# google-research/sparf

Measured on AMD Instinct MI355X. Metric: training rays/sec (64c+128f samples, 8x256 MLP), higher is better.
Workload: dtype bf16x3; 1 GPU; BASELINE configs[1]: DTU-shaped scene, fixed GT poses, photometric loss; 4 views 300x400, 4096 rays x (64 coarse + 128 fine) per GPU and step, fwd+bwd+clip+Adam, both 8x256 MLPs; samples=64+128, precision_mode=bf16x3, launch=eager, optimizer=clip_grad_norm(0.1) + Adam, sparf_amd.optim.FusedAdam

## Files before the change

sparf_amd/csrc/mlp_dev.h:

```cpp
#pragma once
#include <hip/hip_runtime.h>

#include <utility>

#include "streams.h"

namespace sparf {

typedef __bf16 bf16x8 __attribute__((ext_vector_type(8)));
typedef float f32x16 __attribute__((ext_vector_type(16)));
typedef float f32x4 __attribute__((ext_vector_type(4)));
typedef unsigned int u32x4 __attribute__((ext_vector_type(4)));

#define SP_DEV __device__ __forceinline__

template <int N, class F, int... I>
SP_DEV void static_for_impl(F&& f, std::integer_sequence<int, I...>) {
    (f(std::integral_constant<int, I>{}), ...);
}
template <int N, class F> SP_DEV void static_for(F&& f) {
    static_for_impl<N>(static_cast<F&&>(f), std::make_integer_sequence<int, N>{});
}

template <int PREC> struct Policy;

template <> struct Policy<PREC_BF16> {
    enum { PREC = PREC_BF16, KJ = 8, CH = 8, FRAG_BYTES = 1024, LANE_BYTES = 16, G = group_g(PREC_BF16), NWAVES = nwaves_of(PREC_BF16), PREFETCH = 4 };
    typedef bf16x8 B;
    typedef bf16x8 A;
    typedef __bf16 act_t;
    typedef __bf16 stage_t;
    static SP_DEV B zero() { B z; for (int i = 0; i < 8; ++i) z[i] = (__bf16)0.0f; return z; }
    static SP_DEV A lds_frag(const char* p) { return *(const bf16x8*)p; }
    enum { NPART = 1 };
    template <int PART> static SP_DEV f32x16 mfma_part(const A& a, const B& b, f32x16 c) { return __builtin_amdgcn_mfma_f32_32x32x16_bf16(a, b, c, 0, 0, 0); }
    static SP_DEV void set(B* v, int q, float x) { v[q >> 3][q & 7] = (__bf16)x; }
    static SP_DEV float get(const B* v, int q) { return (float)v[q >> 3][q & 7]; }
};

template <> struct Policy<PREC_FP32> {
    enum { PREC = PREC_FP32, KJ = 1, CH = 4, FRAG_BYTES = 256, LANE_BYTES = 4, G = group_g(PREC_FP32), NWAVES = nwaves_of(PREC_FP32), PREFETCH = 4 };
    typedef float B;
    typedef float A;
    typedef float act_t;
    typedef float stage_t;
    static SP_DEV B zero() { return 0.0f; }
    static SP_DEV A lds_frag(const char* p) { return *(const float*)p; }
    enum { NPART = 1 };
    template <int PART> static SP_DEV f32x16 mfma_part(const A& a, const B& b, f32x16 c) { return __builtin_amdgcn_mfma_f32_32x32x2f32(a, b, c, 0, 0, 0); }
    static SP_DEV void set(B* v, int q, float x) { v[q] = x; }
    static SP_DEV float get(const B* v, int q) { return v[q]; }
};

struct bfpair { bf16x8 hi, lo; };
#ifndef SP_X3_PREFETCH
#define SP_X3_PREFETCH 4
#endif
template <> struct Policy<PREC_X3> {
    enum { PREC = PREC_X3, KJ = 8, CH = 8, FRAG_BYTES = 2048, LANE_BYTES = 16, G = group_g(PREC_X3), NWAVES = nwaves_of(PREC_X3), PREFETCH = SP_X3_PREFETCH };
    typedef bfpair B;
    typedef bfpair A;
    typedef __bf16 act_t;
    typedef float stage_t;
    static SP_DEV B zero() { B z; for (int i = 0; i < 8; ++i) { z.hi[i] = (__bf16)0.0f; z.lo[i] = (__bf16)0.0f; } return z; }
    static SP_DEV A lds_frag(const char* p) { A a; a.hi = *(const bf16x8*)p; a.lo = *(const bf16x8*)(p + 1024); return a; }
    enum { NPART = 3 };
    template <int PART> static SP_DEV f32x16 mfma_part(const A& a, const B& b, f32x16 c) {
        if constexpr (PART == 0) return __builtin_amdgcn_mfma_f32_32x32x16_bf16(a.lo, b.hi, c, 0, 0, 0);
        else if constexpr (PART == 1) return __builtin_amdgcn_mfma_f32_32x32x16_bf16(a.hi, b.lo, c, 0, 0, 0);
        else return __builtin_amdgcn_mfma_f32_32x32x16_bf16(a.hi, b.hi, c, 0, 0, 0);
    }
    static SP_DEV void set(B* v, int q, float x) {
        const __bf16 h = (__bf16)x;
        v[q >> 3].hi[q & 7] = h;
        v[q >> 3].lo[q & 7] = (__bf16)(x - (float)h);
    }
    static SP_DEV float get(const B* v, int q) { return (float)v[q >> 3].hi[q & 7] + (float)v[q >> 3].lo[q & 7]; }
};

#ifndef SP_X3_DGRAD_PARTS
#define SP_X3_DGRAD_PARTS 2
#endif
#ifndef SP_X3_DGRAD_WAVES
#define SP_X3_DGRAD_WAVES 0
#endif
template <int W> struct PolicyX3DgradT {
    enum { PREC = PREC_X3, KJ = 8, CH = 8, FRAG_BYTES = 2048, LANE_BYTES = 16, G = group_g(PREC_X3), NWAVES = W,
#ifdef SP_X3_DGRAD_PREFETCH
           PREFETCH = SP_X3_DGRAD_PREFETCH,
#else
           PREFETCH = (W == 8 ? 3 : 4),
#endif
           NPART = SP_X3_DGRAD_PARTS };
    typedef bf16x8 B;
    typedef bfpair A;
    typedef __bf16 act_t;
    typedef float stage_t;
    static SP_DEV B zero() { B z; for (int i = 0; i < 8; ++i) z[i] = (__bf16)0.0f; return z; }
    static SP_DEV A lds_frag(const char* p) { A a; a.hi = *(const bf16x8*)p; a.lo = *(const bf16x8*)(p + 1024); return a; }
    template <int PART> static SP_DEV f32x16 mfma_part(const A& a, const B& b, f32x16 c) {
        if constexpr (PART == 0 && NPART == 2) return __builtin_amdgcn_mfma_f32_32x32x16_bf16(a.lo, b, c, 0, 0, 0);
        else return __builtin_amdgcn_mfma_f32_32x32x16_bf16(a.hi, b, c, 0, 0, 0);
    }
    static SP_DEV void set(B* v, int q, float x) { v[q >> 3][q & 7] = (__bf16)x; }
    static SP_DEV float get(const B* v, int q) { return (float)v[q >> 3][q & 7]; }
};
typedef PolicyX3DgradT<8> PolicyX3Dgrad;
typedef PolicyX3DgradT<4> PolicyX3DgradW4;

#ifdef SP_PROF
struct Prof {
    unsigned long long last, acc[10];
    SP_DEV void start() { for (int i = 0; i < 10; ++i) acc[i] = 0; last = __builtin_amdgcn_s_memtime(); }
    SP_DEV void lap(int k) { const unsigned long long now = __builtin_amdgcn_s_memtime(); acc[k] += now - last; last = now; }
};
#define SP_LAP(prof, k) (prof).lap(k)
#else
struct Prof { SP_DEV void start() {} };
#define SP_LAP(prof, k) ((void)0)
#endif

enum { PIPE_LDS_BYTES = 2 * CHUNK_MAX_BYTES };
#ifdef SP_PROBE_NO_DMA
#define SP_PROBE_NBYTES(x) 0
#else
#define SP_PROBE_NBYTES(x) (x)
#endif

template <int NWAVES, bool SPREAD = false> struct WeightPipe {
    __amdgpu_buffer_rsrc_t rsrc;
    char* lds;
    int wave, lane16;
    unsigned parity;
    Prof prof;

    SP_DEV void init(const char* g, unsigned stream_bytes, char* l) {
        prof.start();
        rsrc = __builtin_amdgcn_make_buffer_rsrc((void*)g, 0, stream_bytes, 0x00020000);
        lane16 = (threadIdx.x & 63) * 16;
        lds = l;
        wave = __builtin_amdgcn_readfirstlane(threadIdx.x >> 6);
        parity = 0;
    }
    SP_DEV void fetch(int off, int bytes, unsigned buf) {
        char* dst = lds + buf * CHUNK_MAX_BYTES;
#pragma unroll
        for (int i = 0; i < CHUNK_MAX_BYTES / (NWAVES * 1024); ++i) {
            int o = (i * NWAVES + wave) * 1024;
            if (o < bytes)
                __builtin_amdgcn_raw_ptr_buffer_load_lds(rsrc, (__attribute__((address_space(3))) void*)(dst + o), 16,
                                                         lane16, off + o, 0, 0);
        }
    }
    template <int OFF, int BYTES, int I> SP_DEV void fetch_piece(unsigned buf) {
        if constexpr (I * NWAVES * 1024 < BYTES) {
            const int o = (I * NWAVES + wave) * 1024;
            if ((I + 1) * NWAVES * 1024 <= BYTES || o < BYTES) {
                __builtin_amdgcn_raw_ptr_buffer_load_lds(rsrc, (__attribute__((address_space(3))) void*)(lds + buf * CHUNK_MAX_BYTES + o), 16,
                                                         lane16, OFF + o, 0, 0);
            }
        }
    }
    enum { PIECES = CHUNK_MAX_BYTES / (NWAVES * 1024), IS_SPREAD = SPREAD };
    SP_DEV void prime(int off, int bytes) { fetch(off, bytes, parity); }
    SP_DEV void drain() { __syncthreads(); }
    template <int NOFF, int NBYTES> SP_DEV const char* acquire() {
#ifndef SP_PROBE_NO_BARRIER
        __syncthreads();
#endif
        SP_LAP(prof, 0);
        if constexpr (!SPREAD)
            static_for<PIECES>([&](auto ic) { this->template fetch_piece<NOFF, NBYTES, decltype(ic)::value>(parity ^ 1u); });
        SP_LAP(prof, 1);
        const char* cur = lds + parity * CHUNK_MAX_BYTES;
        parity ^= 1u;
        return cur;
    }
};

struct NoMid { template <class I, class N> SP_DEV void operator()(I, N) const {} };
#ifndef SP_SPREAD_NUM
#define SP_SPREAD_NUM 3
#define SP_SPREAD_DEN 4
#endif
#ifndef SP_SLOT_BALANCE
#define SP_SLOT_BALANCE 1
#endif
SP_DEV constexpr int last_part_slot(int t, int nmb, int npart) { return (t / nmb) * (npart * nmb) + (npart - 1) * nmb + t % nmb; }
template <class Pipe, int NOFF, int NBYTES, int NMB = 1, int NPART = 1> struct SpreadFetch {
    Pipe& pipe;
    template <class I, class N> SP_DEV void operator()(I, N) const {
        if constexpr (Pipe::IS_SPREAD) {
            constexpr int i = I::value, n = N::value, NP = Pipe::PIECES;
            if constexpr (SP_SLOT_BALANCE && NPART > 1) {
                constexpr int nl = n / NPART, span = SP_SPREAD_NUM * nl / SP_SPREAD_DEN > 0 ? SP_SPREAD_NUM * nl / SP_SPREAD_DEN : 1;
                static_for<NP>([&](auto jc) {
                    constexpr int j = decltype(jc)::value, t0 = j * span / NP, t = t0 < nl ? t0 : nl - 1;
                    if constexpr (last_part_slot(t, NMB, NPART) == i) pipe.template fetch_piece<NOFF, NBYTES, j>(pipe.parity);
                });
            } else {
                constexpr int span = SP_SPREAD_NUM * n / SP_SPREAD_DEN > 0 ? SP_SPREAD_NUM * n / SP_SPREAD_DEN : 1;
                static_for<NP>([&](auto jc) {
                    constexpr int j = decltype(jc)::value, at0 = j * span / NP, at = at0 < n ? at0 : n - 1;
                    if constexpr (at == i) pipe.template fetch_piece<NOFF, NBYTES, j>(pipe.parity);
                });
            }
        }
    }
};
template <class P, int NMB, int NKS, class Mid = NoMid>
SP_DEV void mma_chunk(f32x16 (&acc)[P::G], const typename P::B* b, const char* chunk, int lane, Mid&& mid = Mid{}) {
    constexpr int N = NKS * NMB;
    constexpr int PF = N < P::PREFETCH ? N : P::PREFETCH;
    static_assert(PF >= NMB || N < P::PREFETCH, "the fragments of one k-step are consumed together");
    typename P::A a[PF];
    const char* base = chunk + lane * P::LANE_BYTES;
#pragma unroll
    for (int i = 0; i < PF; ++i) a[i] = P::lds_frag(base + i * P::FRAG_BYTES);
    static_for<NKS>([&](auto kc) {
        constexpr int ks = decltype(kc)::value;
        static_for<P::NPART>([&](auto pc) {
            constexpr int part = decltype(pc)::value;
            static_for<NMB>([&](auto mc) {
                constexpr int m = decltype(mc)::value, i = ks * NMB + m;
                acc[m] = P::template mfma_part<part>(a[i % PF], b[ks], acc[m]);
                if constexpr (part == P::NPART - 1 && i + PF < N) a[i % PF] = P::lds_frag(base + (i + PF) * P::FRAG_BYTES);
                mid(std::integral_constant<int, (ks * P::NPART + part) * NMB + m>{}, std::integral_constant<int, N * P::NPART>{});
                __builtin_amdgcn_sched_barrier(0);
            });
        });
    });
}

SP_DEV constexpr int defer_slot(int p, int np, int ntot) { int at = ((2 * p + 1) * ntot) / (2 * np); return at < ntot ? at : ntot - 1; }
SP_DEV constexpr int defer_first(int gi, int np, int ntot) { int p = 0; while (p < np && defer_slot(p, np, ntot) < gi) ++p; return p; }
template <class P, class Pipe, class Epi, int NMB_PREV, int MB0_PREV, int BASE, int NTOT, int NOFF, int NBYTES, int NMB, int STAGES> struct DeferredEpi {
    Pipe& pipe;
    Epi& epi;
    const f32x16 (&prev)[P::G];
    static constexpr bool BALANCE = SP_SLOT_BALANCE && P::NPART > 1;
    static SP_DEV constexpr int eligible_before(int gi) {
        const int blk = P::NPART * NMB, el = (P::NPART - 1) * NMB, r = gi % blk;
        return BALANCE ? (gi / blk) * el + (r < el ? r : el) : gi;
    }
    template <class I, class N> SP_DEV void operator()(I ic, N nc) const {
        SpreadFetch<Pipe, NOFF, NBYTES, NMB, P::NPART>{pipe}(ic, nc);
        constexpr int gi = BASE + I::value;
        constexpr int NU = NMB_PREV * 8 * STAGES;
        constexpr bool eligible = !BALANCE || (I::value / NMB) % P::NPART != P::NPART - 1;
        if constexpr (eligible) {
            constexpr int e = eligible_before(gi), etot = eligible_before(NTOT);
            constexpr int u0 = defer_first(e, NU, etot), u1 = defer_first(e + 1, NU, etot);
            static_for<u1 - u0>([&](auto uc) {
                constexpr int u = u0 + decltype(uc)::value, p = u / STAGES;
                epi(std::integral_constant<int, MB0_PREV + p / 8>{}, std::integral_constant<int, p % 8>{}, std::integral_constant<int, u % STAGES>{},
                    prev[p / 8], std::true_type{});
            });
        }
    }
};


SP_DEV unsigned lds_addr(const void* p) { return (unsigned)(size_t)(__attribute__((address_space(3))) const char*)p; }
SP_DEV void dma_b32(const void* src, unsigned lds_dst) {
    unsigned keep;
    asm volatile("s_mov_b32 %0, m0\n\ts_mov_b32 m0, %2\n\ts_nop 0\n\tglobal_load_lds_dword %1, off\n\ts_mov_b32 m0, %0"
                 : "=&s"(keep) : "v"(src), "s"(lds_dst) : "memory");
}
SP_DEV void dma_b128(const void* src, unsigned lds_dst) {
    unsigned keep;
    asm volatile("s_mov_b32 %0, m0\n\ts_mov_b32 m0, %2\n\ts_nop 0\n\tglobal_load_lds_dwordx4 %1, off\n\ts_mov_b32 m0, %0"
                 : "=&s"(keep) : "v"(src), "s"(lds_dst) : "memory");
}
enum { STG_ROW_ITEMS = 8, STG_ROW_BYTES = STG_ROW_ITEMS * 256 };
template <class P> struct VencStage {
    enum { EB = (int)sizeof(typename P::stage_t), PIECES = 16 * EB / 16, BYTES = PIECES * 1024, PPC = P::CH * EB / 16 };
    static SP_DEV int src_off(int q, int h) { return ((2 * (q / PPC) + h) * P::CH) * EB + (q % PPC) * 16; }
};
template <class P> SP_DEV void load_chunk(const char* stage, int c, int lane, typename P::B* v) {
    if constexpr (P::PREC == PREC_BF16) {
        v[c] = *(const bf16x8*)(stage + c * 1024 + lane * 16);
    } else if constexpr (P::PREC == PREC_FP32) {
        f32x4 t = *(const f32x4*)(stage + c * 1024 + lane * 16);
        v[4 * c] = t[0]; v[4 * c + 1] = t[1]; v[4 * c + 2] = t[2]; v[4 * c + 3] = t[3];
    } else {
        const f32x4 t0 = *(const f32x4*)(stage + (2 * c) * 1024 + lane * 16), t1 = *(const f32x4*)(stage + (2 * c + 1) * 1024 + lane * 16);
#pragma unroll
        for (int j = 0; j < 4; ++j) { P::set(v, 8 * c + j, t0[j]); P::set(v, 8 * c + 4 + j, t1[j]); }
    }
}

template <class P> SP_DEV __amdgpu_buffer_rsrc_t tile_rsrc(const void* area, int64_t tile32, int64_t tile_bytes, bool in_area = true) {
    return __builtin_amdgcn_make_buffer_rsrc((void*)((const char*)area + (in_area ? tile32 : 0) * tile_bytes), 0, in_area ? (unsigned)tile_bytes : 0u, 0x00020000);
}
SP_DEV int lane_voff(int n, int h) { return n * 16 + h * 512; }
#ifndef SP_SAVE_AUX
#define SP_SAVE_AUX 2
#endif
template <class P, int BASE, int C, int PLANE1> SP_DEV void bstore_chunk(__amdgpu_buffer_rsrc_t r, int voff, const typename P::B* v) {
    constexpr int OFF = BASE + C * 1024;
#ifdef SP_PROBE_HALF_SAVES
    if constexpr (C % 2 == 1) return;
#endif
    if constexpr (sizeof(typename P::B) == 16) {
        __builtin_amdgcn_raw_buffer_store_b128(__builtin_bit_cast(u32x4, v[C]), r, voff, OFF, SP_SAVE_AUX);
    } else if constexpr (P::PREC == PREC_FP32) {
        u32x4 t;
        t[0] = __builtin_bit_cast(unsigned, v[4 * C]); t[1] = __builtin_bit_cast(unsigned, v[4 * C + 1]);
        t[2] = __builtin_bit_cast(unsigned, v[4 * C + 2]); t[3] = __builtin_bit_cast(unsigned, v[4 * C + 3]);
        __builtin_amdgcn_raw_buffer_store_b128(t, r, voff, OFF, SP_SAVE_AUX);
    } else {
        __builtin_amdgcn_raw_buffer_store_b128(__builtin_bit_cast(u32x4, v[C].hi), r, voff, OFF, SP_SAVE_AUX);
// ... 96 lines not shown
```

sparf_amd/csrc/mlp_fwd_impl.h:

```cpp
#pragma once
#include <utility>

#include "kernels.h"
#include "mlp_dev.h"

#if !defined(SP_FWD_PREC) || !defined(SP_FWD_SAVE)
#error "include from mlp_fwd_<precision>_<train|infer>.hip with SP_FWD_PREC / SP_FWD_SAVE defined"
#endif

namespace sparf {

#ifdef SP_PROF
static __device__ unsigned long long g_prof[10];
#endif

enum { EPI_STAGES = 4 };
#ifndef SP_LAZY_ACC_READ
#define SP_LAZY_ACC_READ 1
#endif
template <class P, int L, int NMB> SP_DEV constexpr int group_mfmas_before(int s_end, int kp_end) {
    int n = 0;
    for (int s = 0; s < layer_nseg(L); ++s)
        for (int kp = 0; kp < fwd_seg_nparts(P::PREC, L, s); ++kp) {
            if (s == s_end && kp == kp_end) return n;
// ... 61 lines not shown
    constexpr int AF = area_format(PREC, Q8);
    static_assert(!Q8 || PREC != PREC_FP32, "8-bit saves: bf16-operand modes only");
    typedef typename P::B B;
    typedef typename P::stage_t stage_t;
    constexpr int KJ = P::KJ, CH = P::CH, NW = P::NWAVES;
    constexpr int NB256 = 128 / KJ, NB128 = 64 / KJ, NBX0 = 32 / KJ, NBV = 16 / KJ;
    constexpr int AUX_FLOATS = xyz_exact(PREC) ? AUX_PK_FLOATS : BIAS_PK_FLOATS;
    constexpr bool ROUTED = PREC == PREC_FP32;

    constexpr int C2F_OFF = PIPE_LDS_BYTES + X0_STASH_BYTES + AUX_FLOATS * 4, STG_OFF = C2F_OFF + 64;
    constexpr int STG_WAVE_BYTES = STG_ROW_BYTES + VencStage<P>::BYTES;
    __shared__ __attribute__((aligned(16))) char lds[STG_OFF + NW * STG_WAVE_BYTES];

    const int lane = threadIdx.x & 63, h = lane >> 5, n = lane & 31;
    const int wave = __builtin_amdgcn_readfirstlane(threadIdx.x >> 6);
    constexpr int64_t BIAS_OFF = packed_bias_off(PREC), FWD_OFF = packed_fwd_off(PREC);
    constexpr unsigned FWD_BYTES = (unsigned)fwd_stream_bytes(PREC);
    constexpr int C0_BYTES = chunk_bytes(PREC, fwd_chunk(PREC, 0));
    stage_bias<NW * 64, AUX_FLOATS>((const float*)(a.packed + BIAS_OFF), lds + PIPE_LDS_BYTES + X0_STASH_BYTES);
    const char* bias_pk = lds + PIPE_LDS_BYTES + X0_STASH_BYTES + h * 64;
    float* c2f = (float*)(lds + C2F_OFF);
    if (threadIdx.x < 10) c2f[threadIdx.x] = a.c2f[threadIdx.x];

    typedef WeightPipe<NW, (!SAVE || NW == 4)> Pipe;
    Pipe pipe;
    pipe.init(a.packed + FWD_OFF, FWD_BYTES, lds);
    pipe.prime(0, C0_BYTES);
#ifdef SP_PROBE_NO_DMA
    pipe.fetch(0, C0_BYTES, 1u);
#endif
    __syncthreads();

    const int64_t rows = a.rows;
    const int tile_rows = NW * 32;
    const int64_t ntiles = (rows + tile_rows - 1) / tile_rows;
    const int lvo = lane_voff(n, h);

    char* stg = lds + STG_OFF + wave * STG_WAVE_BYTES;
    const unsigned stg_a = lds_addr(stg);
    auto stage_rows = [&](int64_t tile_n) {
        const int64_t r = (tile_n * NW + wave) * 32 + n;
        const unsigned rc = (unsigned)(r < rows ? r : rows - 1);
        const unsigned ry = rc / (unsigned)a.nsamp;
        ((unsigned*)stg)[7 * 64 + lane] = ry;
        dma_b32(a.t + (ROUTED ? routed_row(rc, a.nsamp, a.row_stride, a.row_off) : (int64_t)rc), stg_a);
#pragma unroll
        for (int j = 0; j < 3; ++j) {
            dma_b32(a.center + 3 * (size_t)ry + j, stg_a + (1 + j) * 256);
            dma_b32(a.dir + 3 * (size_t)ry + j, stg_a + (4 + j) * 256);
        }
    };
    stage_rows(blockIdx.x);
    asm volatile("s_waitcnt vmcnt(0)" ::: "memory");

    for (int64_t tile = blockIdx.x; tile < ntiles; tile += gridDim.x) {
        SP_LAP(pipe.prof, 5);
        const int64_t tile32 = tile * NW + wave;
        const int64_t row = tile32 * 32 + n;
        const bool valid = row < rows;

        const float* sf = (const float*)stg;
        const float tt = sf[lane];
        const float cx = sf[64 + lane], cy = sf[128 + lane], cz = sf[192 + lane];
        const float dx = sf[256 + lane], dy = sf[320 + lane], dz = sf[384 + lane];
        const unsigned ray = ((const unsigned*)stg)[7 * 64 + lane];
        asm volatile("s_waitcnt lgkmcnt(0)" ::: "memory");
        stage_rows(tile + gridDim.x);
        if constexpr (!SAVE) {
            if (a.tile_take != 0) {
                float tmax = -3.0e38f;
#pragma unroll
                for (int w = 0; w < NW; ++w) {
                    const int64_t r = (tile * NW + w) * 32 + 31;
                    tmax = fmaxf(tmax, a.t[r < rows ? r : rows - 1]);
                }
                if ((tmax > a.tile_thr) != (a.tile_take == 2)) {
                    asm volatile("s_waitcnt vmcnt(0)" ::: "memory");
                    continue;
                }
            }
        }
        {
            const char* vrow = (const char*)a.venc + (size_t)ray * (32 * sizeof(stage_t));
#pragma unroll
            for (int q = 0; q < VencStage<P>::PIECES; ++q) dma_b128(vrow + VencStage<P>::src_off(q, h), stg_a + STG_ROW_BYTES + q * 1024);
        }
        SP_LAP(pipe.prof, 6);
        const Xyz pt{__fadd_rn(cx, __fmul_rn(dx, tt)), __fadd_rn(cy, __fmul_rn(dy, tt)), __fadd_rn(cz, __fmul_rn(dz, tt))};
        const float px = pt.x, py = pt.y, pz = pt.z;

        typedef __bf16 bf16x2_t __attribute__((ext_vector_type(2)));
        typedef float f32x2 __attribute__((ext_vector_type(2)));
        char* st = lds + PIPE_LDS_BYTES + wave * (64 * 32 * (int)sizeof(stage_t));
        auto put_pair = [&](int i, float a0, float a1) {
            if constexpr (PREC == PREC_BF16) { const bf16x2_t v = {(__bf16)a0, (__bf16)a1}; ((bf16x2_t*)st)[i * 64 + lane] = v; }
            else { const f32x2 v = {a0, a1}; ((f32x2*)st)[i * 64 + lane] = v; }
        };
        const float pvA = h ? py : px, pvB = h ? pz : py;
        const int split = h ? 5 : 10, kA0 = h ? 5 : 0;
#pragma unroll 1
        for (int i = 0; i < 15; ++i) {
            const bool first = i < split;
            const int k = first ? kA0 + i : i - split;
            const float pv = first ? pvA : pvB;
            const float mk = c2f[k];
            float s, c;
#ifdef SP_PROBE_NO_ENCODING
            s = pv * mk; c = mk;
#else
            sincosf(__fmul_rn(pv, ldexpf(3.14159274101257324219f, k)), &s, &c);
#endif
            put_pair(i, __fmul_rn(s, mk), __fmul_rn(c, mk));
        }
        put_pair(15, h ? pz : px, h ? 0.0f : py);
        SP_LAP(pipe.prof, 7);

        B bx0[NBX0];
        auto load_x0 = [&]() {
            if constexpr (PREC == PREC_BF16) {
#pragma unroll
                for (int c = 0; c < 4; ++c) {
                    u32x4 t;
#pragma unroll
                    for (int j = 0; j < 4; ++j) t[j] = ((const unsigned*)st)[(4 * c + j) * 64 + lane];
                    bx0[c] = __builtin_bit_cast(bf16x8, t);
                }
            } else {
#pragma unroll
                for (int i = 0; i < 16; ++i) {
                    const f32x2 v = ((const f32x2*)st)[i * 64 + lane];
                    P::set(bx0, 2 * i, v[0]);
                    P::set(bx0, 2 * i + 1, v[1]);
                }
            }
        };
        load_x0();
        SP_LAP(pipe.prof, 8);

        __amdgpu_buffer_rsrc_t srs = pipe.rsrc;
        if constexpr (SAVE) srs = tile_rsrc<P>(a.save, tile32, save_tile_bytes(AF));

        B hA[NB256], hB[NB256];

        unsigned mask_bits = 0, e_hi = 0;
        float e_v0 = 0.f, e_v1 = 0.f;
        u32x4 mask_w = {0u, 0u, 0u, 0u};
        auto relu_to = [&](B* out, auto nmbc, auto sbc) {
            return [out, &srs, &mask_w, &mask_bits, &e_hi, &e_v0, &e_v1, lane](auto mbc, auto pairc, auto stagec, const f32x16& acc, auto... deferred) {
                constexpr int mb = decltype(mbc)::value, pr = decltype(pairc)::value, st = decltype(stagec)::value, NMBL = decltype(nmbc)::value;
                constexpr int q0 = 16 * mb + 2 * pr;
                if constexpr (st == 0 || st == 1) {
                    constexpr int r = 2 * pr + st;
                    float x = acc[r];
#if SP_LAZY_ACC_READ
                    if constexpr (sizeof...(deferred) > 0 && NW == 4) asm volatile("v_accvgpr_read_b32 %0, %1" : "=v"(x) : "a"(x));
#endif
                    int yi = __builtin_bit_cast(int, x);
                    yi = yi > 0 ? yi : 0;
                    (st == 0 ? e_v0 : e_v1) = __builtin_bit_cast(float, yi);
                    if constexpr (SAVE)
                        asm("v_cmp_lt_i32 vcc, 0, %1\n\tv_addc_co_u32 %0, vcc, %0, %0, vcc" : "+v"(mask_bits) : "v"(yi) : "vcc");
                } else if constexpr (st == 2) {
                    if constexpr (PREC == PREC_FP32) {
                        out[q0] = e_v0;
                        out[q0 + 1] = e_v1;
                    } else {
                        const bf16x2_t hp = {(__bf16)e_v0, (__bf16)e_v1};
                        e_hi = __builtin_bit_cast(unsigned, hp);
                        if constexpr (PREC == PREC_BF16) {
                            u32x4 t = __builtin_bit_cast(u32x4, out[q0 >> 3]);
                            t[(q0 & 7) >> 1] = e_hi;
                            out[q0 >> 3] = __builtin_bit_cast(bf16x8, t);
                        } else {
                            u32x4 t = __builtin_bit_cast(u32x4, out[q0 >> 3].hi);
                            t[(q0 & 7) >> 1] = e_hi;
                            out[q0 >> 3].hi = __builtin_bit_cast(bf16x8, t);
                            e_v0 -= __builtin_bit_cast(float, e_hi << 16);
                        }
                    }
                } else {
                    if constexpr (PREC == PREC_X3) {
                        e_v1 -= __builtin_bit_cast(float, e_hi & 0xffff0000u);
                        const bf16x2_t lp = {(__bf16)e_v0, (__bf16)e_v1};
                        u32x4 t = __builtin_bit_cast(u32x4, out[q0 >> 3].lo);
                        t[(q0 & 7) >> 1] = __builtin_bit_cast(unsigned, lp);
                        out[q0 >> 3].lo = __builtin_bit_cast(bf16x8, t);
                    }
                    if constexpr (SAVE && pr == 7 && mb % 2 == 1) {
                        mask_w[mb / 2] = mask_bits;
#ifndef SP_PROBE_NO_STORES
                        if constexpr (mb == NMBL - 1)
                            __builtin_amdgcn_raw_buffer_store_b128(mask_w, srs, lane * 16, save_mask_tile_off(AF, decltype(sbc)::value), SP_SAVE_AUX);
#endif
                    }
                }
            };
        };
        typedef std::integral_constant<int, 8> MB8;
        typedef std::integral_constant<int, 4> MB4;
        float qf_a = 0.0f, qf_b = 0.0f;
        auto saver = [&](auto sbc, auto col0c, auto nstc, const B* v, float& qf) {
            return [&srs, &qf, lvo, n, v](auto gc, auto ngc) {
#ifdef SP_PROBE_NO_STORES
                return;
#endif
                constexpr int NST = decltype(nstc)::value, g = decltype(gc)::value, ng = decltype(ngc)::value;
                constexpr int sb = decltype(sbc)::value, col0 = decltype(col0c)::value;
                if constexpr (Q8) {
                    constexpr int N16 = NST / 2, b0 = g * N16 / ng, b1 = (g + 1) * N16 / ng;
                    constexpr int part = col0 >= 256 ? 1 : 0;
                    constexpr bool NONNEG = part == 0;
                    constexpr int BASE = save_buf_tile_off(AF, sb) + (col0 / 32) * 1024;
                    if constexpr (g == 0) {
                        const float amax = q8_amax<NONNEG, NST>(v);
                        qf = q8_factor(amax);
                        q8_store_step<save_step_tile_off(sb, part)>(srs, n, amax);
                    }
                    if constexpr (b1 > b0) static_for<b1 - b0>([&](auto cc) { q8_store16<BASE, b0 + decltype(cc)::value>(srs, lvo, v, qf); });
                } else {
                    constexpr int c0 = g * NST / ng, c1 = (g + 1) * NST / ng;
                    constexpr int BASE = save_buf_tile_off(AF, sb) + (col0 / CH) * 512;
                    if constexpr (SAVE && c1 > c0)
                        static_for<c1 - c0>([&](auto cc) { bstore_chunk<P, BASE, c0 + decltype(cc)::value, (int)save_plane_tile_bytes(AF)>(srs, lvo, v); });
                }
            };
        };
        typedef std::integral_constant<int, 32 / CH> NST_X0;
        typedef std::integral_constant<int, 128 / CH> NST_256;
        typedef std::integral_constant<int, 64 / CH> NST_128;
        typedef std::integral_constant<int, 16 / CH> NST_V;
        typedef std::integral_constant<int, 0> C0;
        typedef std::integral_constant<int, 256> C256;
#define SP_SB(b) std::integral_constant<int, b>{}
#ifndef SP_DEFER_EPI
#define SP_DEFER_EPI 1
#endif
        constexpr bool DEFER = SP_DEFER_EPI;

        { auto e = relu_to(hA, MB8{}, SP_SB(SB_H0)); fwd_layer<P, 0, DEFER, Pipe>(pipe, bias_pk, lane, bx0, bx0, e, saver(SP_SB(SB_XS), C256{}, NST_X0{}, bx0, qf_a), pt); }
        { auto e = relu_to(hB, MB8{}, SP_SB(SB_H1)); fwd_layer<P, 1, DEFER, Pipe>(pipe, bias_pk, lane, hA, hA, e, saver(SP_SB(SB_H0), C0{}, NST_256{}, hA, qf_a)); }
        { auto e = relu_to(hA, MB8{}, SP_SB(SB_H2)); fwd_layer<P, 2, DEFER, Pipe>(pipe, bias_pk, lane, hB, hB, e, saver(SP_SB(SB_H1), C0{}, NST_256{}, hB, qf_a)); }
        { auto e = relu_to(hB, MB8{}, SP_SB(SB_XS)); fwd_layer<P, 3, DEFER, Pipe>(pipe, bias_pk, lane, hA, hA, e, saver(SP_SB(SB_H2), C0{}, NST_256{}, hA, qf_a)); }
        load_x0();
        { auto e = relu_to(hA, MB8{}, SP_SB(SB_H4)); fwd_layer<P, 4, DEFER, Pipe>(pipe, bias_pk, lane, hB, bx0, e, saver(SP_SB(SB_XS), C0{}, NST_256{}, hB, qf_a), pt); }
        { auto e = relu_to(hB, MB8{}, SP_SB(SB_H5)); fwd_layer<P, 5, DEFER, Pipe>(pipe, bias_pk, lane, hA, hA, e, saver(SP_SB(SB_H4), C0{}, NST_256{}, hA, qf_a)); }
        { auto e = relu_to(hA, MB8{}, SP_SB(SB_H6)); fwd_layer<P, 6, DEFER, Pipe>(pipe, bias_pk, lane, hB, hB, e, saver(SP_SB(SB_H5), C0{}, NST_256{}, hB, qf_a)); }

        float raw_sigma = 0.0f;
        {
            auto relu7 = relu_to(hB, MB8{}, SP_SB(SB_FV));
            auto epi7 = [&](auto mbc, auto pairc, auto stagec, const f32x16& acc, auto... deferred) {
                constexpr int mb = decltype(mbc)::value;
                if constexpr (mb < 8) relu7(mbc, pairc, stagec, acc, deferred...);
                else if constexpr (decltype(pairc)::value == 0 && decltype(stagec)::value == 0) raw_sigma = acc[0];
            };
            fwd_layer<P, 7, DEFER, Pipe>(pipe, bias_pk, lane, hA, hA, epi7, saver(SP_SB(SB_H6), C0{}, NST_256{}, hA, qf_a));
        }
        if (valid && h == 0) a.sigma_raw[ROUTED ? routed_row(row, a.nsamp, a.row_stride, a.row_off) : row] = raw_sigma;

        B bv[NBV];
        {
#pragma unroll
            for (int c = 0; c < 16 / CH; ++c) load_chunk<P>(stg + STG_ROW_BYTES, c, lane, bv);
        }
        B gv[NB128];
        {
            auto s_feat = saver(SP_SB(SB_FV), C0{}, NST_256{}, hB, qf_a);
            auto s_view = saver(SP_SB(SB_FV), C256{}, NST_V{}, bv, qf_b);
            auto e = relu_to(gv, MB4{}, SP_SB(SB_G));
            fwd_layer<P, 8, DEFER, Pipe>(pipe, bias_pk, lane, hB, bv, e, [&](auto gc, auto ngc) { s_feat(gc, ngc); s_view(gc, ngc); });
        }
        float z0 = 0.f, z1 = 0.f, z2 = 0.f;
        {
            auto epi9 = [&](auto, auto pairc, auto stagec, const f32x16& acc, auto...) {
                if constexpr (decltype(stagec)::value == 0) {
                    if constexpr (decltype(pairc)::value == 0) { z0 = acc[0]; z1 = acc[1]; }
                    else if constexpr (decltype(pairc)::value == 1) z2 = acc[2];
                }
            };
            fwd_layer<P, 9, false, Pipe>(pipe, bias_pk, lane, gv, gv, epi9, saver(SP_SB(SB_G), C0{}, NST_128{}, gv, qf_a));
        }
#undef SP_SB
        SP_LAP(pipe.prof, 9);
#ifdef SP_PROBE_NO_TILE_END
        if (valid && h == 0 && z0 + z1 + z2 == 12345.678f) a.rgb[row * 3] = z0;
#else
        if (valid && h == 0) {
            float* o = a.rgb + (ROUTED ? routed_row(row, a.nsamp, a.row_stride, a.row_off) : row) * 3;
            o[0] = 1.0f / (1.0f + expf(-z0));
            o[1] = 1.0f / (1.0f + expf(-z1));
            o[2] = 1.0f / (1.0f + expf(-z2));
        }
#endif
    }
    asm volatile("s_waitcnt vmcnt(0)" ::: "memory");
    pipe.drain();
#ifdef SP_PROF
    SP_LAP(pipe.prof, 5);
    if (blockIdx.x == 0 && threadIdx.x == 0)
        for (int i = 0; i < 10; ++i) g_prof[i] = pipe.prof.acc[i];
#endif
}

int SP_FWD_LAUNCHER(const MlpFwdArgs& a, int grid, hipStream_t stream) {
    if (a.rows <= 0) return 0;
    hipLaunchKernelGGL((mlp_fwd_kernel<SP_FWD_PREC, (int)SP_FWD_SAVE>), dim3(grid), dim3(Policy<SP_FWD_PREC>::NWAVES * 64), 0, stream, a);
    return hipGetLastError() == hipSuccess ? 0 : 2;
}

}

#if defined(SP_PROF) && SP_FWD_PROF_EXPORT
extern "C" int sparf_debug_prof(unsigned long long* out) {
    return hipMemcpyFromSymbol(out, HIP_SYMBOL(sparf::g_prof), 10 * sizeof(unsigned long long)) == hipSuccess ? 0 : 1;
}
// ... 2 lines not shown
```

sparf_amd/csrc/wgrad.hip:

```cpp
#include <type_traits>

#include "kernels.h"
#include "mlp_dev.h"

namespace sparf {

enum { WG_THREADS = 512, WGRAD_LDS_BYTES = 160 * 1024 };
#ifndef SP_WG_NT
#define SP_WG_NT " nt"
#endif
#ifndef SP_WG_SPREAD
#define SP_WG_SPREAD 0
#endif

template <int PREC> struct WOps;
template <> struct WOps<PREC_BF16> {
    static SP_DEV float fsum(bf16x8 v) {
        float s = 0.f;
#pragma unroll
        for (int j = 0; j < 8; ++j) s += (float)v[j];
        return s;
    }
};
template <> struct WOps<PREC_FP32> {
// ... 219 lines not shown
            if constexpr (decltype(widec)::value)
                asm volatile("s_mov_b32 %0, m0\n\ts_mov_b32 m0, %2\n\ts_nop 0\n\tglobal_load_lds_dwordx4 %1, off" SP_WG_NT "\n\ts_mov_b32 m0, %0"
                             : "=&s"(keep) : "v"(src), "s"(lds_dst) : "memory");
            else
                asm volatile("s_mov_b32 %0, m0\n\ts_mov_b32 m0, %2\n\ts_nop 0\n\tglobal_load_lds_dword %1, off" SP_WG_NT "\n\ts_mov_b32 m0, %0"
                             : "=&s"(keep) : "v"(src), "s"(lds_dst) : "memory");
        };
        auto issue_q8_op = [&](int t, int k) {
            const int64_t tile32 = (r_begin >> 5) + t;
            if (k < QP_HI) {
                char* slot = ring8 + (t % QD) * QSLOT;
                const int p = k * 8 + wave;
                if (p < PQ) {
                    const bool is_x = p >= MB;
                    const int C = is_x ? p - MB : p;
                    dma((is_x ? xq + tile32 * XQ_TILE : dyq + tile32 * DYQ_TILE) + C * 1024 + lane * 16, slot + p * 1024, std::true_type{});
                }
            } else {
                char* sw = steps + (t % QD) * SSLOT + wave * 512;
                if (k == QP_HI) dma(dys + tile32 * DYQ_TILE + lane * 4, sw, std::false_type{});
                else dma(xs + tile32 * XQ_TILE + lane * 4, sw + 256, std::false_type{});
            }
        };
        auto issue_q8 = [&](int t) {
#pragma unroll
            for (int k = 0; k < QP_HI + 2; ++k) issue_q8_op(t, k);
        };
        auto convert_q8 = [&](int t, char* dst) {
            const char* slot = ring8 + (t % QD) * QSLOT;
            const char* sw = steps + (t % QD) * SSLOT + wave * 512;
#pragma unroll
            for (int i = 0; i < QP_HI; ++i) {
                const int p = i * 8 + wave;
                if (p < PQ) {
                    const bool is_x = p >= MB;
                    const int C = is_x ? p - MB : p;
                    const int part = (is_x ? jb.xcol0 / 32 + C : mb0 + C) >= 8 ? 1 : 0;
                    const u32x4 q = *(const u32x4*)(slot + p * 1024 + lane * 16);
                    const float step = *(const float*)(sw + (is_x ? 256 : 0) + part * 128 + row * 4), off = -128.0f * step;
                    typedef __bf16 bf16x2_t __attribute__((ext_vector_type(2)));
                    u32x4 o[2];
#pragma unroll
                    for (int j = 0; j < 4; ++j) {
                        const unsigned w = q[j];
                        const bf16x2_t lo = {(__bf16)fmaf((float)(w & 0xffu), step, off), (__bf16)fmaf((float)((w >> 8) & 0xffu), step, off)};
                        const bf16x2_t hi = {(__bf16)fmaf((float)((w >> 16) & 0xffu), step, off), (__bf16)fmaf((float)(w >> 24), step, off)};
                        o[j >> 1][2 * (j & 1)] = __builtin_bit_cast(unsigned, lo);
                        o[j >> 1][2 * (j & 1) + 1] = __builtin_bit_cast(unsigned, hi);
                    }
                    char* region = dst + (is_x ? DY_BYTES : 0);
                    const int k0 = 4 * C + h, k1 = k0 + 2;
                    *(u32x4*)(region + k0 * CS + ((row ^ ((k0 & 3) << 2)) << 4)) = o[0];
                    *(u32x4*)(region + k1 * CS + ((row ^ ((k1 & 3) << 2)) << 4)) = o[1];
                }
            }
        };
        for (int t = 0; t < QD && t < ntiles; ++t) issue_q8(t);
        for (int t = 0; t < ntiles; ++t) {
            const int ahead = ntiles - 1 - t < QD - 1 ? ntiles - 1 - t : QD - 1;
            static_for<QD>([&](auto ac) {
                constexpr int A = decltype(ac)::value;
                if (ahead == A) {
                    if (wave < QN_HI) asm volatile("s_waitcnt vmcnt(%0)" ::"n"(A * (QP_HI + 2)) : "memory");
                    else asm volatile("s_waitcnt vmcnt(%0)" ::"n"(A * (QP_LO + 2)) : "memory");
                }
            });
            char* buf = lds + (t & 1) * BUF_BYTES;
            convert_q8(t, buf);
            asm volatile("s_waitcnt lgkmcnt(0)" ::: "memory");
            if constexpr (SP_WG_SPREAD) {
                asm volatile("s_barrier" ::: "memory");
                const bool refill = t + QD < ntiles;
                compute_tile(buf, [&](int i) {
#pragma unroll
                    for (int k = 0; k < QP_HI + 2; ++k)
                        if (i == k * NS / (QP_HI + 2) && refill) issue_q8_op(t + QD, k);
                });
            } else {
                if (t + QD < ntiles) issue_q8(t + QD);
                asm volatile("s_barrier" ::: "memory");
                compute_tile(buf, [](int) {});
            }
        }
    }

    float* out = a.partial + (int64_t)blockIdx.x * WPARTIAL;
    float* mat = out + wjob_mat_off(job);
#pragma unroll
    for (int j = 0; j < NJ; ++j) {
        const int m = N_OWNER ? j : fix_blk;
        const int nb_raw = N_OWNER ? wave : wave / MB + WPM * j;
        if (nb_raw < NB) {
#pragma unroll
            for (int r = 0; r < 16; ++r) {
                const int po = 32 * (m + mb0) + (r & 3) + 8 * (r >> 2) + 4 * h;
                mat[(int64_t)po * N + nb_raw * 32 + (lane & 31)] = acc[j][r];
            }
        }
    }
    float* bo = out + wjob_bias_off(job);
#pragma unroll
    for (int b = 0; b < NBIAS; ++b) {
        const int m = N_OWNER ? wave + 8 * b : wave;
        const float sum = bsum[b] + __shfl_xor(bsum[b], 32);
        if (m < MB && lane < 32) bo[32 * (m + mb0) + lane] = sum;
    }
}

template <int PREC, bool Q8, int MB, int NB> SP_DEV void wgrad_dispatch(const WgradArgs& a, int job, char* lds) {
    if constexpr (Q8) {
        static_assert(PREC != PREC_FP32, "8-bit areas: bf16-operand modes");
        wgrad_job_dma<MB, NB, 1, 32, 2, true>(a, job, lds);
    } else if constexpr (PREC == PREC_BF16) {
        wgrad_job_dma<MB, NB>(a, job, lds);
    } else if constexpr (PREC == PREC_X3) {
#ifndef SP_WG_X3_ROWS
#define SP_WG_X3_ROWS 16
#endif
        if constexpr (nplanes_of(PREC_X3) == 2) wgrad_job_dma<MB, NB, 2, SP_WG_X3_ROWS>(a, job, lds);
        else wgrad_job_dma<MB, NB>(a, job, lds);
    } else {
        wgrad_job_dma<MB, NB, 1, 16, 4>(a, job, lds);
    }
}

#ifndef SP_WG_Q8_HALVES
#define SP_WG_Q8_HALVES 0
#endif
enum { WGRAD_H_LDS_BYTES = 80 * 1024 };
enum : unsigned { WGRAD_H_JOBS = (1u << 0) | (1u << 1) | (1u << 2) | (1u << 3) | (1u << 5) | (1u << 6) };
__global__ void __launch_bounds__(WG_THREADS, 4) wgrad_q8h_kernel(WgradArgs a) {
    __shared__ __attribute__((aligned(16))) char lds[WGRAD_H_LDS_BYTES];
    const int job = blockIdx.y, mb0 = 4 * (int)blockIdx.z;
    if (!((WGRAD_H_JOBS >> job) & 1u)) return;
    if (job == 0) wgrad_job_dma<4, 2, 1, 32, 2, true, WGRAD_H_LDS_BYTES>(a, job, lds, mb0);
    else wgrad_job_dma<4, 8, 1, 32, 2, true, WGRAD_H_LDS_BYTES>(a, job, lds, mb0);
}

template <int PREC, bool Q8 = false>
__global__ void __launch_bounds__(WG_THREADS) wgrad_kernel(WgradArgs a, unsigned job_mask) {
    __shared__ __attribute__((aligned(16))) char lds[WGRAD_LDS_BYTES];
    const int job = blockIdx.y;
    if (!((job_mask >> job) & 1u)) return;
    switch (job) {
        case 0: wgrad_dispatch<PREC, Q8, 8, 2>(a, job, lds); break;
        case 4: wgrad_dispatch<PREC, Q8, 8, 10>(a, job, lds); break;
        case 7: wgrad_dispatch<PREC, Q8, 9, 8>(a, job, lds); break;
        case 8: wgrad_dispatch<PREC, Q8, 4, 9>(a, job, lds); break;
        case 9: wgrad_dispatch<PREC, Q8, 1, 4>(a, job, lds); break;
        default: wgrad_dispatch<PREC, Q8, 8, 8>(a, job, lds); break;
    }
}

__global__ void wgrad_reduce_kernel(const float* __restrict__ partial, int nsplit, const int32_t* __restrict__ wsrc,
                                    float* __restrict__ out, int accumulate) {
    int p = blockIdx.x * blockDim.x + threadIdx.x;
    if (p >= N_PARAMS) return;
    constexpr int64_t WPARTIAL = wpartial_floats();
    const int64_t src = wsrc[p];
    float s = 0.f;
    for (int k = 0; k < nsplit; ++k) s += partial[(int64_t)k * WPARTIAL + src];
    out[p] = accumulate ? out[p] + s : s;
}

int launch_wgrad_partials(int prec, bool q8, const WgradArgs& a, int nsplit, hipStream_t s) {
    if (a.rows <= 0 || nsplit <= 0) return 1;
    dim3 grid(nsplit, N_WJOBS), block(WG_THREADS);
    const unsigned all = ~0u;
    if (q8) {
        if (prec != PREC_BF16 && prec != PREC_X3) return 1;
        if (SP_WG_Q8_HALVES) {
            hipLaunchKernelGGL(wgrad_q8h_kernel, dim3(nsplit, N_WJOBS, 2), block, 0, s, a);
            hipLaunchKernelGGL((wgrad_kernel<PREC_BF16, true>), grid, block, 0, s, a, all & ~(unsigned)WGRAD_H_JOBS);
        } else hipLaunchKernelGGL((wgrad_kernel<PREC_BF16, true>), grid, block, 0, s, a, all);
    } else if (prec == PREC_BF16) hipLaunchKernelGGL(wgrad_kernel<PREC_BF16>, grid, block, 0, s, a, all);
    else if (prec == PREC_X3) hipLaunchKernelGGL(wgrad_kernel<PREC_X3>, grid, block, 0, s, a, all);
    else if (prec == PREC_FP32) hipLaunchKernelGGL(wgrad_kernel<PREC_FP32>, grid, block, 0, s, a, all);
    else return 1;
    return hipGetLastError() == hipSuccess ? 0 : 2;
}
int launch_wgrad_reduce(const float* partial, int nsplit, const int32_t* wsrc, float* grad_out, hipStream_t s, bool accumulate) {
    hipLaunchKernelGGL(wgrad_reduce_kernel, dim3((N_PARAMS + 255) / 256), dim3(256), 0, s, partial, nsplit, wsrc, grad_out, accumulate ? 1 : 0);
    return hipGetLastError() == hipSuccess ? 0 : 2;
}
int launch_wgrad(int prec, bool q8, const WgradArgs& a, int nsplit, const int32_t* wsrc, float* grad_out, hipStream_t s, bool accumulate) {
    const int rc = launch_wgrad_partials(prec, q8, a, nsplit, s);
    return rc ? rc : launch_wgrad_reduce(a.partial, nsplit, wsrc, grad_out, s, accumulate);
}

}
```

Baseline: 621,200 rays/s.

## Fold wave offset into buffer rsrc, fuse lazy ReLU asm, batch wgrad reduce loads

```diff
diff --git a/sparf_amd/csrc/mlp_dev.h b/sparf_amd/csrc/mlp_dev.h
--- a/sparf_amd/csrc/mlp_dev.h
+++ b/sparf_amd/csrc/mlp_dev.h
@@ -130,34 +130,35 @@
 template <int NWAVES, bool SPREAD = false> struct WeightPipe {
     __amdgpu_buffer_rsrc_t rsrc;
     char* lds;
+    char* lds_w;
     int wave, lane16;
     unsigned parity;
     Prof prof;
 
     SP_DEV void init(const char* g, unsigned stream_bytes, char* l) {
         prof.start();
-        rsrc = __builtin_amdgcn_make_buffer_rsrc((void*)g, 0, stream_bytes, 0x00020000);
+        wave = __builtin_amdgcn_readfirstlane(threadIdx.x >> 6);
+        rsrc = __builtin_amdgcn_make_buffer_rsrc((void*)(g + wave * 1024), 0, stream_bytes - wave * 1024, 0x00020000);
         lane16 = (threadIdx.x & 63) * 16;
         lds = l;
-        wave = __builtin_amdgcn_readfirstlane(threadIdx.x >> 6);
+        lds_w = l + wave * 1024;
         parity = 0;
     }
     SP_DEV void fetch(int off, int bytes, unsigned buf) {
-        char* dst = lds + buf * CHUNK_MAX_BYTES;
+        char* dst = lds_w + buf * CHUNK_MAX_BYTES;
 #pragma unroll
         for (int i = 0; i < CHUNK_MAX_BYTES / (NWAVES * 1024); ++i) {
-            int o = (i * NWAVES + wave) * 1024;
-            if (o < bytes)
-                __builtin_amdgcn_raw_ptr_buffer_load_lds(rsrc, (__attribute__((address_space(3))) void*)(dst + o), 16,
-                                                         lane16, off + o, 0, 0);
+            if ((i * NWAVES + wave) * 1024 < bytes)
+                __builtin_amdgcn_raw_ptr_buffer_load_lds(rsrc, (__attribute__((address_space(3))) void*)(dst + i * NWAVES * 1024), 16,
+                                                         lane16, off + i * NWAVES * 1024, 0, 0);
         }
     }
     template <int OFF, int BYTES, int I> SP_DEV void fetch_piece(unsigned buf) {
         if constexpr (I * NWAVES * 1024 < BYTES) {
-            const int o = (I * NWAVES + wave) * 1024;
-            if ((I + 1) * NWAVES * 1024 <= BYTES || o < BYTES) {
-                __builtin_amdgcn_raw_ptr_buffer_load_lds(rsrc, (__attribute__((address_space(3))) void*)(lds + buf * CHUNK_MAX_BYTES + o), 16,
-                                                         lane16, OFF + o, 0, 0);
+            constexpr int O = I * NWAVES * 1024;
+            if ((I + 1) * NWAVES * 1024 <= BYTES || wave * 1024 < BYTES - O) {
+                __builtin_amdgcn_raw_ptr_buffer_load_lds(rsrc, (__attribute__((address_space(3))) void*)(lds_w + buf * CHUNK_MAX_BYTES + O), 16,
+                                                         lane16, OFF + O, 0, 0);
             }
         }
     }
diff --git a/sparf_amd/csrc/mlp_fwd_impl.h b/sparf_amd/csrc/mlp_fwd_impl.h
--- a/sparf_amd/csrc/mlp_fwd_impl.h
+++ b/sparf_amd/csrc/mlp_fwd_impl.h
@@ -237,15 +237,22 @@
                 if constexpr (st == 0 || st == 1) {
                     constexpr int r = 2 * pr + st;
                     float x = acc[r];
-#if SP_LAZY_ACC_READ
-                    if constexpr (sizeof...(deferred) > 0 && NW == 4) asm volatile("v_accvgpr_read_b32 %0, %1" : "=v"(x) : "a"(x));
-#endif
-                    int yi = __builtin_bit_cast(int, x);
-                    yi = yi > 0 ? yi : 0;
+                    int yi;
+                    constexpr bool LAZY = SP_LAZY_ACC_READ && sizeof...(deferred) > 0 && NW == 4;
+                    if constexpr (LAZY && SAVE) {
+                        asm volatile("v_accvgpr_read_b32 %0, %2\n\tv_max_i32 %0, 0, %0\n\tv_cmp_lt_i32 vcc, 0, %0\n\tv_addc_co_u32 %1, vcc, %1, %1, vcc"
+                                     : "=v"(yi), "+v"(mask_bits) : "a"(x) : "vcc");
+                    } else if constexpr (LAZY) {
+                        asm volatile("v_accvgpr_read_b32 %0, %1\n\tv_max_i32 %0, 0, %0" : "=v"(yi) : "a"(x));
+                    } else {
+                        yi = __builtin_bit_cast(int, x);
+                        yi = yi > 0 ? yi : 0;
+                        if constexpr (SAVE)
+                            asm("v_cmp_lt_i32 vcc, 0, %1\n\tv_addc_co_u32 %0, vcc, %0, %0, vcc" : "+v"(mask_bits) : "v"(yi) : "vcc");
+                    }
                     (st == 0 ? e_v0 : e_v1) = __builtin_bit_cast(float, yi);
-                    if constexpr (SAVE)
-                        asm("v_cmp_lt_i32 vcc, 0, %1\n\tv_addc_co_u32 %0, vcc, %0, %0, vcc" : "+v"(mask_bits) : "v"(yi) : "vcc");
                 } else if constexpr (st == 2) {
+                    if constexpr (SP_LAZY_ACC_READ && sizeof...(deferred) > 0 && NW == 4) __builtin_amdgcn_sched_barrier(0);
                     if constexpr (PREC == PREC_FP32) {
                         out[q0] = e_v0;
                         out[q0 + 1] = e_v1;
diff --git a/sparf_amd/csrc/wgrad.hip b/sparf_amd/csrc/wgrad.hip
--- a/sparf_amd/csrc/wgrad.hip
+++ b/sparf_amd/csrc/wgrad.hip
@@ -395,14 +395,23 @@
     }
 }
 
-__global__ void wgrad_reduce_kernel(const float* __restrict__ partial, int nsplit, const int32_t* __restrict__ wsrc,
-                                    float* __restrict__ out, int accumulate) {
+enum { RED_AHEAD = 16 };
+__global__ void __launch_bounds__(256) wgrad_reduce_kernel(const float* __restrict__ partial, int nsplit, const int32_t* __restrict__ wsrc,
+                                                           float* __restrict__ out, int accumulate) {
     int p = blockIdx.x * blockDim.x + threadIdx.x;
     if (p >= N_PARAMS) return;
     constexpr int64_t WPARTIAL = wpartial_floats();
-    const int64_t src = wsrc[p];
+    const float* src = partial + wsrc[p];
     float s = 0.f;
-    for (int k = 0; k < nsplit; ++k) s += partial[(int64_t)k * WPARTIAL + src];
+    int k = 0;
+    for (; k + RED_AHEAD <= nsplit; k += RED_AHEAD) {
+        float v[RED_AHEAD];
+#pragma unroll
+        for (int j = 0; j < RED_AHEAD; ++j) v[j] = src[(int64_t)(k + j) * WPARTIAL];
+#pragma unroll
+        for (int j = 0; j < RED_AHEAD; ++j) s += v[j];
+    }
+    for (; k < nsplit; ++k) s += src[(int64_t)k * WPARTIAL];
     out[p] = accumulate ? out[p] + s : s;
 }
 
```

Result: faster. 632,800 rays/s (median of 6 runs) (+1.9%).
